# leo27945875/Python_Stable_3D_Truss_Analysis

Measured on AMD Instinct MI355X. Metric: truss solves/sec (batched Solve), higher is better.
Workload: dtype f64; 1 GPU; bar-942_input_0 x 4096 independent copies per GPU (nJ 244, nM 942, n_free 696); batch_per_gpu=4096, parallelism=batch-sharded x1, no collective

## Files before the change

### python_stable_3d_truss_analysis_amd/csrc/recover.hip

```cpp
#include "trs_common.h"
#include "../../include/trs_solver.h"
#include "trs_recover.h"

namespace {

using namespace trs_rec;

#define TRS_RECOVER_LIST_CAP 32768

template <bool STAGED>
__global__ __launch_bounds__(256) void trs_recover_kernel(
    const double* __restrict__ xyz, const TrsMembers mem, const double* __restrict__ loads,
    const int* __restrict__ free_index, const int* __restrict__ nJ, const int* __restrict__ nM,
    const int nJ_max, const int nM_max, const double* __restrict__ uf, const int ld_uf,
    double* __restrict__ u_out, double* __restrict__ f_out, double* __restrict__ N_out,
    const int* __restrict__ joint_out,
    const long long* __restrict__ out_rows, const int nJ_out, const int nM_out, const int* __restrict__ info_in,
    int* __restrict__ info_out, const int scan_only) {
    extern __shared__ double sh[];
    const int b = blockIdx.x, tid = threadIdx.x;
    const int joints = nJ[b];
    const int ndof = 3 * joints, ndof_max = 3 * nJ_max;
    const size_t orow = out_rows != nullptr ? (size_t)out_rows[b] : (size_t)b;
    const size_t odof = out_rows != nullptr ? (size_t)3 * nJ_out : (size_t)ndof_max;
    const size_t omem = out_rows != nullptr ? (size_t)nM_out : (size_t)nM_max;
    if (out_rows != nullptr && tid == 0 && info_out != nullptr) info_out[orow] = info_in[b];
    double *u, *f;
    if constexpr (STAGED) {
        u = sh;
        f = sh + ndof_max;
    } else {
        u = u_out + orow * odof;
        f = f_out + orow * odof;
    }
    int* cnt = reinterpret_cast<int*>(sh + 2 * ndof_max);
    int* start = cnt + nJ_max;
    int* ends = start + nJ_max + 1;
    unsigned char* held = reinterpret_cast<unsigned char*>(ends + 2 * nM_max);
    const int* fi = free_index + (size_t)b * ndof_max;
    const double* F = loads + (size_t)b * ndof_max;
    const double* ufb = uf + (size_t)b * ld_uf;
    const int members = nM[b];
    constexpr int MR = 4;
    int2 cjr[MR];
    const size_t mbase = (size_t)b * nM_max;
    auto CNI = [&](int m) { return mem.ends(mbase + m); };
#pragma unroll
    for (int r = 0; r < MR; ++r) {
        const int m = tid + 256 * r;
        cjr[r] = m < members ? CNI(m) : int2{0, 0};
    }
    const int* jo = joint_out ? joint_out + (size_t)b * nJ_max : nullptr;
    auto J = [&](int j) { return (!STAGED && jo) ? jo[j] : j; };
    for (int d = tid; d < ndof_max; d += 256) {
        const int r = d < ndof ? fi[d] : -1;
        const int o = 3 * J(d / 3) + d % 3;
        u[o] = r >= 0 ? ufb[r] : 0.0;
        f[o] = r >= 0 ? F[d] : 0.0;
    }
    if constexpr (STAGED)
        for (int j = tid; j < nJ_max; j += 256) {
            cnt[j] = 0;
            held[j] = j < joints ? (unsigned char)((fi[3 * j] < 0) | (fi[3 * j + 1] < 0) | (fi[3 * j + 2] < 0)) : (unsigned char)0;
        }
    if constexpr (!STAGED) __threadfence();
    __syncthreads();
    const double* X = xyz + (size_t)b * ndof_max;
    auto constrained = [&](int j) {
        if constexpr (STAGED) return (int)held[j];
        else return (fi[3 * j] < 0) | (fi[3 * j + 1] < 0) | (fi[3 * j + 2] < 0);
    };
    auto slot = [&](int j) {
        const int a0 = fi[3 * j] < 0 ? 0 : (fi[3 * j + 1] < 0 ? 1 : 2);
        return reinterpret_cast<int*>(&f[3 * J(j) + a0]);
    };
    auto slot_get = [&](int j, int k) { return __hip_atomic_load(slot(j) + k, __ATOMIC_RELAXED, __HIP_MEMORY_SCOPE_WORKGROUP); };
    auto slot_set = [&](int j, int k, int v) { __hip_atomic_store(slot(j) + k, v, __ATOMIC_RELAXED, __HIP_MEMORY_SCOPE_WORKGROUP); };
    auto ends_of = [&](int r, int m) {
        int2 c = CNI(m < members ? m : 0);
#pragma unroll
        for (int q = 0; q < MR; ++q)
            if (r == q) c = cjr[q];
        return c;
    };
    for (int m = tid, r = 0; m < nM_max; m += 256, ++r) {
        const size_t mm = (size_t)b * nM_max + m;
        double axial = 0.0;
        if (m < members) {
            const int2 c = r < MR ? ends_of(r, m) : CNI(m);
            const int j0 = c.x, j1 = c.y;
            const MemberGeom g = member_geom(X, j0, j1);
            axial = member_axial(g, mem.EA(mm), u, J(j0), J(j1));
            if constexpr (STAGED) {
                if (constrained(j0)) atomicAdd(&cnt[j0], 1);
                if (constrained(j1)) atomicAdd(&cnt[j1], 1);
            } else {
                if (constrained(j0)) atomicAdd(slot(j0), 1);
                if (constrained(j1)) atomicAdd(slot(j1), 1);
            }
        }
        N_out[orow * omem + m] = axial;
    }
    if constexpr (STAGED) {
        __syncthreads();
        if (tid < 64) {
            int base = 0;
            for (int j0 = 0; j0 < joints; j0 += 64) {
                const int j = j0 + tid;
                const int v = j < joints ? cnt[j] : 0;
                int incl = v;
#pragma unroll
                for (int off = 1; off < 64; off <<= 1) {
                    const int up = __shfl_up(incl, off);
                    if (tid >= off) incl += up;
                }
                if (j < joints) start[j] = base + incl - v;
                base += __shfl(incl, 63);
            }
        }
        __syncthreads();
        for (int j = tid; j < joints; j += 256) cnt[j] = 0;
        __syncthreads();
        for (int m = tid, r = 0; m < members; m += 256, ++r) {
            const int2 c = r < MR ? ends_of(r, m) : CNI(m);
            const int j0 = c.x, j1 = c.y;
            if (constrained(j0)) ends[start[j0] + atomicAdd(&cnt[j0], 1)] = m << 1;
            if (constrained(j1)) ends[start[j1] + atomicAdd(&cnt[j1], 1)] = (m << 1) | 1;
        }
        __syncthreads();
        for (int j = tid; j < joints; j += 256) {
            const int deg = cnt[j];
            if (deg == 0) continue;
            double r[3];
            joint_reaction(ends + start[j], deg, mem, X, mbase, u, nullptr, r);
#pragma unroll
            for (int a = 0; a < 3; ++a)
                if (fi[3 * j + a] < 0) f[3 * j + a] = r[a];
        }
        __syncthreads();
        if (jo != nullptr) {
            int* inv = cnt;
            for (int j = tid; j < nJ_max; j += 256) inv[jo[j]] = j;
            __syncthreads();
            for (int o = tid; o < ndof_max; o += 256) {
                const int d = 3 * inv[o / 3] + o % 3;
                u_out[orow * odof + o] = u[d];
                f_out[orow * odof + o] = d < ndof ? f[d] : 0.0;
            }
        } else {
            for (int d = tid; d < ndof_max; d += 256) {
                u_out[orow * odof + d] = u[d];
                f_out[orow * odof + d] = d < ndof ? f[d] : 0.0;
            }
        }
    } else {
        int* lists = reinterpret_cast<int*>(sh);
        int* wsum = lists + TRS_RECOVER_LIST_CAP;
        __threadfence();
        __syncthreads();
        int base = 0;
        for (int j0 = 0; j0 < joints; j0 += 256) {
            const int j = j0 + tid;
            const bool own = j < joints && constrained(j);
            const int v = own ? slot_get(j, 0) : 0;
            int incl = v;
#pragma unroll
            for (int off = 1; off < 64; off <<= 1) {
                const int up = __shfl_up(incl, off);
                if ((tid & 63) >= off) incl += up;
            }
            if ((tid & 63) == 63) wsum[tid >> 6] = incl;
            __syncthreads();
            int before = 0, total = 0;
#pragma unroll
            for (int w = 0; w < 4; ++w) {
                before += w < (tid >> 6) ? wsum[w] : 0;
                total += wsum[w];
            }
            if (own) {
                slot_set(j, 1, base + before + incl - v);
                slot_set(j, 0, 0);
            }
            base += total;
            __syncthreads();
        }
        __threadfence();
        __syncthreads();
        if (base <= TRS_RECOVER_LIST_CAP && scan_only == 0) {
            for (int m = tid, r = 0; m < members; m += 256, ++r) {
                const int2 c = r < MR ? ends_of(r, m) : CNI(m);
                const int j0 = c.x, j1 = c.y;
                if (constrained(j0)) lists[slot_get(j0, 1) + atomicAdd(slot(j0), 1)] = m << 1;
                if (constrained(j1)) lists[slot_get(j1, 1) + atomicAdd(slot(j1), 1)] = (m << 1) | 1;
            }
            __threadfence();
            __syncthreads();
            for (int j = tid; j < joints; j += 256) {
                if (!constrained(j)) continue;
                double r[3];
                joint_reaction(lists + slot_get(j, 1), slot_get(j, 0), mem, X, mbase, u, jo, r);
#pragma unroll
                for (int a = 0; a < 3; ++a)
                    if (fi[3 * j + a] < 0) f[3 * J(j) + a] = r[a];
            }
        } else {
            const int wave = tid >> 6, lane = tid & 63;
            for (int j = wave; j < joints; j += 4) {
                if (!constrained(j)) continue;
                double r[3] = {0.0, 0.0, 0.0};
                for (int m0 = 0; m0 < members; m0 += 64) {
                    const int m = m0 + lane;
                    const int2 c = m < members ? CNI(m) : int2{-1, -1};
                    const bool h0 = c.x == j, h1 = c.y == j;
                    const unsigned long long b0 = __ballot(h0), b1 = __ballot(h1);
                    unsigned long long any = b0 | b1;
                    if (any == 0ull) continue;
                    double axial = 0.0, cc[3] = {0.0, 0.0, 0.0};
                    if (h0 || h1) {
                        const MemberGeom g = member_geom(X, c.x, c.y);
                        const size_t mm = (size_t)b * nM_max + m;
                        axial = member_axial(g, mem.EA(mm), u, J(c.x), J(c.y));
#pragma unroll
                        for (int a = 0; a < 3; ++a) cc[a] = g.c[a];
                    }
                    while (any != 0ull) {
                        const int src = __builtin_ctzll(any);
                        any &= any - 1;
                        const double ax = __shfl(axial, src);
                        const double cs[3] = {__shfl(cc[0], src), __shfl(cc[1], src), __shfl(cc[2], src)};
                        if ((b0 >> src) & 1ull) add_end_force(r, cs, ax, 0);
                        if ((b1 >> src) & 1ull) add_end_force(r, cs, ax, 1);
                    }
                }
                if (lane == 0) {
#pragma unroll
                    for (int a = 0; a < 3; ++a)
                        if (fi[3 * j + a] < 0) f[3 * J(j) + a] = r[a];
                }
            }
        }
    }
}

__device__ __forceinline__ double block_sum(double v, double* red) {
#pragma unroll
    for (int off = 32; off > 0; off >>= 1) v += __shfl_down(v, off);
    if ((threadIdx.x & 63) == 0) red[threadIdx.x >> 6] = v;
    __syncthreads();
    const double total = red[0] + red[1] + red[2] + red[3];
    __syncthreads();
    return total;
}

__global__ __launch_bounds__(256) void trs_fitness_kernel(
    const double* __restrict__ xyz, const int* __restrict__ conn, const double* __restrict__ A,
    const double* __restrict__ rho, const int* __restrict__ nJ, const int* __restrict__ nM,
    const int nJ_max, const int nM_max, const double* __restrict__ u, const double* __restrict__ N,
    const double allow_stress, const double allow_displace, double* __restrict__ weight,
    double* __restrict__ stress_vio, double* __restrict__ disp_vio) {
    __shared__ double red[4];
    const int b = blockIdx.x, tid = threadIdx.x;
    const double* X = xyz + (size_t)b * 3 * nJ_max;
    double w = 0.0, sv = 0.0, dv = 0.0;
    for (int m = tid; m < nM[b]; m += 256) {
        const size_t mm = (size_t)b * nM_max + m;
        const MemberGeom g = member_geom(X, conn[2 * mm], conn[2 * mm + 1]);
        w += A[mm] * g.len * rho[mm];
        const double force = N[mm];
        if (fabs(force) >= 1e-10) {
            const double s = fabs(force) / A[mm];
            if (s > allow_stress) sv += s - allow_stress;
        }
    }
    const double* U = u + (size_t)b * 3 * nJ_max;
    for (int j = tid; j < nJ[b]; j += 256) {
        const double ux = U[3 * j], uy = U[3 * j + 1], uz = U[3 * j + 2];
        if (fabs(ux) >= 1e-10 || fabs(uy) >= 1e-10 || fabs(uz) >= 1e-10) {
            const double l = sqrt(ux * ux + uy * uy + uz * uz);
            if (l > allow_displace) dv += l - allow_displace;
        }
    }
    w = block_sum(w, red);
    sv = block_sum(sv, red);
    dv = block_sum(dv, red);
    if (tid == 0) {
        weight[b] = w;
        stress_vio[b] = sv;
        disp_vio[b] = dv;
    }
}

}

extern "C" int trs_recover_launch(int B, int nJ_max, int nM_max, const double* xyz, const TrsMembers* members,
                                  const double* loads,
                                  const int* free_index, const int* nJ, const int* nM,
                                  const double* uf, int ld_uf, double* u, double* f_ext, double* N,
                                  const int* joint_out, int force_unstaged, hipStream_t stream,
                                  const long long* out_rows, int nJ_out, int nM_out, const int* info_in,
                                  int* info_out) {
    if (B <= 0) return 0;
    const size_t lds = ((size_t)6 * nJ_max * sizeof(double) +
                        ((size_t)2 * nJ_max + 1 + 2 * (size_t)nM_max) * sizeof(int) + (size_t)nJ_max + 15) / 16 * 16;
    if (lds > 160 * 1024 || force_unstaged) {
        const size_t lds_lists = (size_t)(TRS_RECOVER_LIST_CAP + 8) * sizeof(int);
        static const int lists_limit_set = (int)hipFuncSetAttribute(
            reinterpret_cast<const void*>(trs_recover_kernel<false>), hipFuncAttributeMaxDynamicSharedMemorySize,
            160 * 1024);
        (void)lists_limit_set;
        hipLaunchKernelGGL(trs_recover_kernel<false>, dim3(B), dim3(256), lds_lists, stream, xyz, *members, loads,
                           free_index, nJ, nM, nJ_max, nM_max, uf, ld_uf, u, f_ext, N, joint_out, out_rows, nJ_out,
                           nM_out, info_in, info_out, (force_unstaged & TRS_HINT_RECOVER_SCAN) != 0);
        return (int)hipGetLastError();
    }
    static const int lds_limit_set = (int)hipFuncSetAttribute(
        reinterpret_cast<const void*>(trs_recover_kernel<true>), hipFuncAttributeMaxDynamicSharedMemorySize,
        160 * 1024);
    (void)lds_limit_set;
    hipLaunchKernelGGL(trs_recover_kernel<true>, dim3(B), dim3(256), lds, stream, xyz, *members, loads,
                       free_index, nJ, nM, nJ_max, nM_max, uf, ld_uf, u, f_ext, N, joint_out, out_rows, nJ_out, nM_out,
                       info_in, info_out, 0);
    return (int)hipGetLastError();
}

__global__ __launch_bounds__(256) void trs_ga_sections_kernel(
    const unsigned char* __restrict__ genes, const double* __restrict__ table, const int count, const int n_member,
    const int n_type, const int nM_max, const long long total, double* __restrict__ A, double* __restrict__ E,
    double* __restrict__ rho) {
    const long long i = (long long)blockIdx.x * 256 + threadIdx.x;
    if (i >= total) return;
    const int b = (int)(i / nM_max), m = (int)(i - (long long)b * nM_max);
    const int type = (b < count && m < n_member) ? (int)genes[(size_t)b * n_member + m] : 0;
    const bool ok = type < n_type;
    const double nan = __builtin_nan("");
    A[i] = ok ? table[3 * type] : nan;
    E[i] = ok ? table[3 * type + 1] : nan;
    rho[i] = ok ? table[3 * type + 2] : nan;
}

extern "C" int trs_ga_sections_launch(int B, int nM_max, int count, int n_member, int n_type, const unsigned char* genes,
                                      const double* table, double* A, double* E, double* rho, hipStream_t stream) {
    const long long total = (long long)B * nM_max;
    if (total <= 0) return 0;
    hipLaunchKernelGGL(trs_ga_sections_kernel, dim3((unsigned)((total + 255) / 256)), dim3(256), 0, stream, genes, table,
                       count, n_member, n_type, nM_max, total, A, E, rho);
    return (int)hipGetLastError();
}

extern "C" int trs_fitness_launch(int B, int nJ_max, int nM_max, const double* xyz, const int* conn,
                                  const double* A, const double* rho, const int* nJ, const int* nM,
                                  const double* u, const double* N, double allow_stress,
                                  double allow_displace, double* weight, double* stress_vio,
                                  double* disp_vio, hipStream_t stream) {
    if (B <= 0) return 0;
    hipLaunchKernelGGL(trs_fitness_kernel, dim3(B), dim3(256), 0, stream, xyz, conn, A, rho, nJ, nM,
                       nJ_max, nM_max, u, N, allow_stress, allow_displace, weight, stress_vio,
                       disp_vio);
    return (int)hipGetLastError();
}
```

Before: 2.803 million solves/s.

## Restructure staged recover kernel to fuse axial and end-list passes with LDS stash

Moves the staged recover path into a separate device function. It fuses the member axial-force pass with building the per-joint end lists, using atomicSub on a precomputed prefix scan so one member pass is removed. Axial force and direction cosines for the first list slots are stashed in LDS, so joint reactions can be summed without recomputing member geometry; entries are insertion-sorted to keep summation order deterministic. It also shrinks the end indices to 16-bit, batches member loads two at a time, and adds an occupancy hint to launch bounds. The cost is extra code complexity and a cap on member count for the staged path.

```diff
diff --git a/python_stable_3d_truss_analysis_amd/csrc/recover.hip b/python_stable_3d_truss_analysis_amd/csrc/recover.hip
--- a/python_stable_3d_truss_analysis_amd/csrc/recover.hip
+++ b/python_stable_3d_truss_analysis_amd/csrc/recover.hip
@@ -8,8 +8,221 @@
 
 #define TRS_RECOVER_LIST_CAP 32768
 
+constexpr int STAGED_MEMBERS_MAX = 32768;
+constexpr int STASH_CAP = 64;
+struct StagedLds {
+    size_t u, f, stash, cnt, start, ends, held, total;
+};
+__host__ __device__ inline StagedLds staged_lds(int nJ_max, int nM_max) {
+    StagedLds l;
+    size_t p = 0;
+    auto take = [&](size_t bytes) { const size_t at = p; p += bytes; return at; };
+    l.u = take((size_t)3 * nJ_max * sizeof(double));
+    l.f = take((size_t)3 * nJ_max * sizeof(double));
+    l.stash = take((size_t)STASH_CAP * 4 * sizeof(double));
+    l.cnt = take((size_t)nJ_max * sizeof(int));
+    l.start = take(((size_t)nJ_max + 1) * sizeof(int));
+    l.ends = take((size_t)2 * nM_max * sizeof(unsigned short));
+    l.held = take((size_t)nJ_max);
+    l.total = (p + 15) / 16 * 16;
+    return l;
+}
+
+template <bool TABLE>
+__device__ __forceinline__ void recover_staged(
+    double* sh, const int b, const int tid, const double* __restrict__ xyz, const TrsMembers& batch_members,
+    const double* __restrict__ loads, const int* __restrict__ free_index, const int joints, const int members,
+    const int nJ_max, const int nM_max, const double* __restrict__ ufb, double* __restrict__ u_row,
+    double* __restrict__ f_row, double* __restrict__ N_row, const int* __restrict__ jo) {
+    const int ndof = 3 * joints, ndof_max = 3 * nJ_max;
+    const StagedLds lay = staged_lds(nJ_max, nM_max);
+    unsigned char* base = reinterpret_cast<unsigned char*>(sh);
+    double* u = reinterpret_cast<double*>(base + lay.u);
+    double* f = reinterpret_cast<double*>(base + lay.f);
+    double* stash = reinterpret_cast<double*>(base + lay.stash);
+    int* cnt = reinterpret_cast<int*>(base + lay.cnt);
+    int* start = reinterpret_cast<int*>(base + lay.start);
+    unsigned short* ends = reinterpret_cast<unsigned short*>(base + lay.ends);
+    unsigned char* held = base + lay.held;
+    const size_t mbase = (size_t)b * nM_max;
+    TrsMembers mem = batch_members;
+    mem.conn = static_cast<const char*>(mem.conn) + mbase * (TABLE ? sizeof(ushort2) : sizeof(int2));
+    if constexpr (TABLE) {
+        mem.tidx += mbase;
+    } else {
+        mem.E += mbase;
+        mem.A += mbase;
+    }
+    const double* X = xyz + (size_t)b * ndof_max;
+    constexpr int MR = 4;
+    int2 cjr[MR];
+    auto ends_at = [&](int m) {
+        if constexpr (TABLE) {
+            const ushort2 c = static_cast<const ushort2*>(mem.conn)[(unsigned)m];
+            return int2{(int)c.x, (int)c.y};
+        } else {
+            return static_cast<const int2*>(mem.conn)[(unsigned)m];
+        }
+    };
+#pragma unroll
+    for (int r = 0; r < MR; ++r) cjr[r] = int2{0, 0};
+    if (members > 0) {
+#pragma unroll
+        for (int r = 0; r < MR; ++r) cjr[r] = ends_at(min(tid + 256 * r, members - 1));
+    }
+    auto ends_of = [&](int r, int m) {
+        int2 c = r < MR ? int2{0, 0} : ends_at(m);
+#pragma unroll
+        for (int q = 0; q < MR; ++q)
+            if (r == q) c = cjr[q];
+        return c;
+    };
+    const int jo_first = (jo != nullptr && tid < nJ_max) ? jo[tid] : 0;
+    {
+        const int* fi = free_index + (size_t)b * ndof_max;
+        const double* F = loads + (size_t)b * ndof_max;
+        for (int j = tid; j < nJ_max; j += 256) {
+            int r[3];
+            double load[3], sol[3];
+#pragma unroll
+            for (int a = 0; a < 3; ++a) {
+                r[a] = j < joints ? fi[3 * j + a] : -1;
+                load[a] = F[3 * j + a];
+            }
+#pragma unroll
+            for (int a = 0; a < 3; ++a) sol[a] = r[a] >= 0 ? ufb[r[a]] : 0.0;
+#pragma unroll
+            for (int a = 0; a < 3; ++a) {
+                u[3 * j + a] = r[a] >= 0 ? sol[a] : 0.0;
+                f[3 * j + a] = r[a] >= 0 ? load[a] : 0.0;
+            }
+            cnt[j] = 0;
+            held[j] = j < joints ? (unsigned char)((r[0] < 0) | ((r[1] < 0) << 1) | ((r[2] < 0) << 2)) : (unsigned char)0;
+        }
+    }
+    __syncthreads();
+    for (int m = tid, r = 0; m < members; m += 256, ++r) {
+        const int2 c = ends_of(r, m);
+        if (held[c.x]) atomicAdd(&cnt[c.x], 1);
+        if (held[c.y]) atomicAdd(&cnt[c.y], 1);
+    }
+    __syncthreads();
+    if (tid < 64) {
+        int total = 0;
+        for (int j0 = 0; j0 < joints; j0 += 64) {
+            const int j = j0 + tid;
+            const int v = j < joints ? cnt[j] : 0;
+            int incl = v;
+#pragma unroll
+            for (int off = 1; off < 64; off <<= 1) {
+                const int up = __shfl_up(incl, off);
+                if (tid >= off) incl += up;
+            }
+            if (j < joints) start[j] = total + incl - v;
+            total += __shfl(incl, 63);
+        }
+        if (tid == 0) start[joints] = total;
+    }
+    __syncthreads();
+    for (int m = members + tid; m < nM_max; m += 256) N_row[m] = 0.0;
+    constexpr int MB = 2;
+    for (int m0 = tid, r0 = 0; m0 < members; m0 += MB * 256, r0 += MB) {
+        int2 c[MB];
+        double xl[MB][6], se[MB], sa[MB];
+#pragma unroll
+        for (int q = 0; q < MB; ++q) {
+            const int m = min(m0 + 256 * q, members - 1);
+            c[q] = ends_of(r0 + q, m);
+            if constexpr (TABLE) {
+                const double* t = mem.types + 3 * (int)mem.tidx[(unsigned)m];
+                se[q] = t[1];
+                sa[q] = t[0];
+            } else {
+                se[q] = mem.E[(unsigned)m];
+                sa[q] = mem.A[(unsigned)m];
+            }
+#pragma unroll
+            for (int a = 0; a < 3; ++a) {
+                xl[q][a] = X[3u * (unsigned)c[q].x + a];
+                xl[q][3 + a] = X[3u * (unsigned)c[q].y + a];
+            }
+        }
+#pragma unroll
+        for (int q = 0; q < MB; ++q) {
+            const int m = m0 + 256 * q;
+            if (m >= members) continue;
+            const int j0 = c[q].x, j1 = c[q].y;
+            const MemberGeom g = member_geom(xl[q], 0, 1);
+            const double axial = member_axial(g, se[q] * sa[q], u, j0, j1);
+            auto list_end = [&](int j, int end) {
+                if (!held[j]) return;
+                const int slot = start[j] + atomicSub(&cnt[j], 1) - 1;
+                ends[slot] = (unsigned short)((m << 1) | end);
+                if (slot < STASH_CAP) {
+                    stash[4 * slot] = axial;
+#pragma unroll
+                    for (int a = 0; a < 3; ++a) stash[4 * slot + 1 + a] = g.c[a];
+                }
+            };
+            list_end(j0, 0);
+            list_end(j1, 1);
+            N_row[m] = axial;
+        }
+    }
+    __syncthreads();
+    for (int j = tid; j < joints; j += 256) {
+        const int s = start[j], deg = start[j + 1] - s, axes = held[j];
+        if (deg == 0) continue;
+        double r[3];
+        if (s + deg <= STASH_CAP) {
+            unsigned short* list = ends + s;
+            double* rec = stash + 4 * s;
+            for (int i = 1; i < deg; ++i) {
+                const int key = list[i];
+                const double k0 = rec[4 * i], k1 = rec[4 * i + 1], k2 = rec[4 * i + 2], k3 = rec[4 * i + 3];
+                int p = i - 1;
+                while (p >= 0 && list[p] > key) {
+                    list[p + 1] = list[p];
+#pragma unroll
+                    for (int a = 0; a < 4; ++a) rec[4 * (p + 1) + a] = rec[4 * p + a];
+                    --p;
+                }
+                list[p + 1] = (unsigned short)key;
+                rec[4 * (p + 1)] = k0; rec[4 * (p + 1) + 1] = k1; rec[4 * (p + 1) + 2] = k2; rec[4 * (p + 1) + 3] = k3;
+            }
+            r[0] = r[1] = r[2] = 0.0;
+            for (int i = 0; i < deg; ++i) {
+                const double cs[3] = {rec[4 * i + 1], rec[4 * i + 2], rec[4 * i + 3]};
+                add_end_force(r, cs, rec[4 * i], list[i] & 1);
+            }
+        } else {
+            joint_reaction(ends + s, deg, mem, X, 0, u, nullptr, r);
+        }
+#pragma unroll
+        for (int a = 0; a < 3; ++a)
+            if ((axes >> a) & 1) f[3 * j + a] = r[a];
+    }
+    if (jo != nullptr) {
+        int* inv = cnt;
+        if (tid < nJ_max) inv[jo_first] = tid;
+        for (int j = tid + 256; j < nJ_max; j += 256) inv[jo[j]] = j;
+        __syncthreads();
+        for (int o = tid; o < ndof_max; o += 256) {
+            const int d = 3 * inv[o / 3] + o % 3;
+            u_row[o] = u[d];
+            f_row[o] = d < ndof ? f[d] : 0.0;
+        }
+    } else {
+        __syncthreads();
+        for (int d = tid; d < ndof_max; d += 256) {
+            u_row[d] = u[d];
+            f_row[d] = d < ndof ? f[d] : 0.0;
+        }
+    }
+}
+
 template <bool STAGED>
-__global__ __launch_bounds__(256) void trs_recover_kernel(
+__global__ __launch_bounds__(256, STAGED ? 8 : 1) void trs_recover_kernel(
     const double* __restrict__ xyz, const TrsMembers mem, const double* __restrict__ loads,
     const int* __restrict__ free_index, const int* __restrict__ nJ, const int* __restrict__ nM,
     const int nJ_max, const int nM_max, const double* __restrict__ uf, const int ld_uf,
@@ -25,18 +238,18 @@
     const size_t odof = out_rows != nullptr ? (size_t)3 * nJ_out : (size_t)ndof_max;
     const size_t omem = out_rows != nullptr ? (size_t)nM_out : (size_t)nM_max;
     if (out_rows != nullptr && tid == 0 && info_out != nullptr) info_out[orow] = info_in[b];
-    double *u, *f;
+    const int* jo = joint_out ? joint_out + (size_t)b * nJ_max : nullptr;
     if constexpr (STAGED) {
-        u = sh;
-        f = sh + ndof_max;
-    } else {
-        u = u_out + orow * odof;
-        f = f_out + orow * odof;
-    }
-    int* cnt = reinterpret_cast<int*>(sh + 2 * ndof_max);
-    int* start = cnt + nJ_max;
-    int* ends = start + nJ_max + 1;
-    unsigned char* held = reinterpret_cast<unsigned char*>(ends + 2 * nM_max);
+        if (mem.table())
+            recover_staged<true>(sh, b, tid, xyz, mem, loads, free_index, joints, nM[b], nJ_max, nM_max, uf + (size_t)b * ld_uf,
+                                 u_out + orow * odof, f_out + orow * odof, N_out + orow * omem, jo);
+        else
+            recover_staged<false>(sh, b, tid, xyz, mem, loads, free_index, joints, nM[b], nJ_max, nM_max, uf + (size_t)b * ld_uf,
+                                  u_out + orow * odof, f_out + orow * odof, N_out + orow * omem, jo);
+        return;
+    }
+    double* u = u_out + orow * odof;
+    double* f = f_out + orow * odof;
     const int* fi = free_index + (size_t)b * ndof_max;
     const double* F = loads + (size_t)b * ndof_max;
     const double* ufb = uf + (size_t)b * ld_uf;
@@ -50,26 +263,17 @@
         const int m = tid + 256 * r;
         cjr[r] = m < members ? CNI(m) : int2{0, 0};
     }
-    const int* jo = joint_out ? joint_out + (size_t)b * nJ_max : nullptr;
-    auto J = [&](int j) { return (!STAGED && jo) ? jo[j] : j; };
+    auto J = [&](int j) { return jo ? jo[j] : j; };
     for (int d = tid; d < ndof_max; d += 256) {
         const int r = d < ndof ? fi[d] : -1;
         const int o = 3 * J(d / 3) + d % 3;
         u[o] = r >= 0 ? ufb[r] : 0.0;
         f[o] = r >= 0 ? F[d] : 0.0;
     }
-    if constexpr (STAGED)
-        for (int j = tid; j < nJ_max; j += 256) {
-            cnt[j] = 0;
-            held[j] = j < joints ? (unsigned char)((fi[3 * j] < 0) | (fi[3 * j + 1] < 0) | (fi[3 * j + 2] < 0)) : (unsigned char)0;
-        }
-    if constexpr (!STAGED) __threadfence();
+    __threadfence();
     __syncthreads();
     const double* X = xyz + (size_t)b * ndof_max;
-    auto constrained = [&](int j) {
-        if constexpr (STAGED) return (int)held[j];
-        else return (fi[3 * j] < 0) | (fi[3 * j + 1] < 0) | (fi[3 * j + 2] < 0);
-    };
+    auto constrained = [&](int j) { return (fi[3 * j] < 0) | (fi[3 * j + 1] < 0) | (fi[3 * j + 2] < 0); };
     auto slot = [&](int j) {
         const int a0 = fi[3 * j] < 0 ? 0 : (fi[3 * j + 1] < 0 ? 1 : 2);
         return reinterpret_cast<int*>(&f[3 * J(j) + a0]);
@@ -91,69 +295,12 @@
             const int j0 = c.x, j1 = c.y;
             const MemberGeom g = member_geom(X, j0, j1);
             axial = member_axial(g, mem.EA(mm), u, J(j0), J(j1));
-            if constexpr (STAGED) {
-                if (constrained(j0)) atomicAdd(&cnt[j0], 1);
-                if (constrained(j1)) atomicAdd(&cnt[j1], 1);
-            } else {
-                if (constrained(j0)) atomicAdd(slot(j0), 1);
-                if (constrained(j1)) atomicAdd(slot(j1), 1);
-            }
+            if (constrained(j0)) atomicAdd(slot(j0), 1);
+            if (constrained(j1)) atomicAdd(slot(j1), 1);
         }
         N_out[orow * omem + m] = axial;
     }
-    if constexpr (STAGED) {
-        __syncthreads();
-        if (tid < 64) {
-            int base = 0;
-            for (int j0 = 0; j0 < joints; j0 += 64) {
-                const int j = j0 + tid;
-                const int v = j < joints ? cnt[j] : 0;
-                int incl = v;
-#pragma unroll
-                for (int off = 1; off < 64; off <<= 1) {
-                    const int up = __shfl_up(incl, off);
-                    if (tid >= off) incl += up;
-                }
-                if (j < joints) start[j] = base + incl - v;
-                base += __shfl(incl, 63);
-            }
-        }
-        __syncthreads();
-        for (int j = tid; j < joints; j += 256) cnt[j] = 0;
-        __syncthreads();
-        for (int m = tid, r = 0; m < members; m += 256, ++r) {
-            const int2 c = r < MR ? ends_of(r, m) : CNI(m);
-            const int j0 = c.x, j1 = c.y;
-            if (constrained(j0)) ends[start[j0] + atomicAdd(&cnt[j0], 1)] = m << 1;
-            if (constrained(j1)) ends[start[j1] + atomicAdd(&cnt[j1], 1)] = (m << 1) | 1;
-        }
-        __syncthreads();
-        for (int j = tid; j < joints; j += 256) {
-            const int deg = cnt[j];
-            if (deg == 0) continue;
-            double r[3];
-            joint_reaction(ends + start[j], deg, mem, X, mbase, u, nullptr, r);
-#pragma unroll
-            for (int a = 0; a < 3; ++a)
-                if (fi[3 * j + a] < 0) f[3 * j + a] = r[a];
-        }
-        __syncthreads();
-        if (jo != nullptr) {
-            int* inv = cnt;
-            for (int j = tid; j < nJ_max; j += 256) inv[jo[j]] = j;
-            __syncthreads();
-            for (int o = tid; o < ndof_max; o += 256) {
-                const int d = 3 * inv[o / 3] + o % 3;
-                u_out[orow * odof + o] = u[d];
-                f_out[orow * odof + o] = d < ndof ? f[d] : 0.0;
-            }
-        } else {
-            for (int d = tid; d < ndof_max; d += 256) {
-                u_out[orow * odof + d] = u[d];
-                f_out[orow * odof + d] = d < ndof ? f[d] : 0.0;
-            }
-        }
-    } else {
+    {
         int* lists = reinterpret_cast<int*>(sh);
         int* wsum = lists + TRS_RECOVER_LIST_CAP;
         __threadfence();
@@ -300,9 +447,8 @@
                                   const long long* out_rows, int nJ_out, int nM_out, const int* info_in,
                                   int* info_out) {
     if (B <= 0) return 0;
-    const size_t lds = ((size_t)6 * nJ_max * sizeof(double) +
-                        ((size_t)2 * nJ_max + 1 + 2 * (size_t)nM_max) * sizeof(int) + (size_t)nJ_max + 15) / 16 * 16;
-    if (lds > 160 * 1024 || force_unstaged) {
+    const size_t lds = staged_lds(nJ_max, nM_max).total;
+    if (lds > 160 * 1024 || nM_max > STAGED_MEMBERS_MAX || force_unstaged) {
         const size_t lds_lists = (size_t)(TRS_RECOVER_LIST_CAP + 8) * sizeof(int);
         static const int lists_limit_set = (int)hipFuncSetAttribute(
             reinterpret_cast<const void*>(trs_recover_kernel<false>), hipFuncAttributeMaxDynamicSharedMemorySize,
```

Result: slower. 2.721 million solves/s (-2.9%).
